# mlpc-ucsd/BDM

Hardware: AMD Instinct MI355X
Metric: sampled shapes/sec (4096 pts, 1000 DDPM steps) (higher is better)
Workload: dtype f32

## Files before the change

bdm_amd/csrc/pvconv_compact.hip:

```cpp
#include <stdlib.h>

#include "../../include/bdm_hip.h"
#include "common.h"
#include "se_fc.h"

using namespace bdm;

typedef __attribute__((ext_vector_type(8))) _Float16 f16x8;

namespace {

__device__ __forceinline__ void split2c(float v, unsigned short &h, unsigned short &l) {
  v = fminf(fmaxf(v, -65504.f), 65504.f);
  const _Float16 hi = (_Float16)v;
  const _Float16 lo = (_Float16)(v - (float)hi);
  h = __builtin_bit_cast(unsigned short, hi);
  l = __builtin_bit_cast(unsigned short, lo);
}

__device__ __forceinline__ void split_rec(const float v[8], uint4 &ph, uint4 &pl) {
  unsigned short h[8], l[8];
#pragma unroll
  for (int j = 0; j < 8; ++j) split2c(v[j], h[j], l[j]);
  ph.x = h[0] | (h[1] << 16); ph.y = h[2] | (h[3] << 16); ph.z = h[4] | (h[5] << 16); ph.w = h[6] | (h[7] << 16);
  pl.x = l[0] | (l[1] << 16); pl.y = l[2] | (l[3] << 16); pl.z = l[4] | (l[5] << 16); pl.w = l[6] | (l[7] << 16);
}

__device__ __forceinline__ void all_group_stats(const double *__restrict__ partial, int bi, int G, int S, double count, float eps,
                                                float *s_mean, float *s_rstd) {
  const int tid = threadIdx.x, l = tid & 31, gq = tid >> 5, per = blockDim.x >> 5;
  for (int g0 = 0; g0 < G; g0 += per) {
    const int g = g0 + gq;
    double a = 0.0, q = 0.0;
    if (g < G) {
      const double *pp = partial + ((size_t)bi * G + g) * S * 2;
      for (int sl = l; sl < S; sl += 32) { a += pp[2 * sl]; q += pp[2 * sl + 1]; }
    }
    a = half32_sum(a); q = half32_sum(q);
    if (l == 0 && g < G) {
      const double mu = a / count;
      double var = q / count - mu * mu;
      if (var < 0) var = 0;
      s_mean[g] = (float)mu;
      s_rstd[g] = (float)(1.0 / sqrt(var + (double)eps));
    }
  }
  __syncthreads();
}

}

__global__ __launch_bounds__(256) void to_h2_rows_kernel(int C, int V, int G, int S, int n_rows_max, int tiles_max, int dense_in,
                                                         const float *__restrict__ x, const int *__restrict__ dil_list,
                                                         const int *__restrict__ tile_start, const float *__restrict__ bias,
                                                         const double *__restrict__ partial, const float *__restrict__ gamma,
                                                         const float *__restrict__ beta, float eps, int act, float act_scale,
                                                         uint4 *__restrict__ rows_h2, uint4 *__restrict__ const_h2,
                                                         float *__restrict__ const_f32, unsigned *__restrict__ saturated) {
  __shared__ float s_mean[64], s_rstd[64];
  __shared__ float s_a[256], s_b[256];
  const int bi = blockIdx.y, tid = threadIdx.x, lane = tid & 63;
  const int C8 = (C + 7) / 8;
  const int nd = tile_start[((size_t)bi * tiles_max + tiles_max - 1) * 16 + 1];
  constexpr int RB = 512;
  if ((int)blockIdx.x * RB >= nd && blockIdx.x != 0) return;
  const int cg = C / G;
  const float g_pre = tid < C ? gamma[tid] : 0.f, b_pre = tid < C ? beta[tid] : 0.f;
  const int per_pass = blockDim.x / C8;
  const int c8 = tid % C8, rl = tid / C8;
  const int nch = min(8, C - c8 * 8);
  const bool vec = (C & 3) == 0 && nch == 8;
  auto load_row = [&](int j, float (&in)[8]) {
    if (dense_in) {
      const int v = dil_list[(size_t)bi * n_rows_max + j];
      const float *xb = x + ((size_t)bi * C + c8 * 8) * V + v;
#pragma unroll
      for (int u = 0; u < 8; ++u) in[u] = xb[(size_t)min(u, nch - 1) * V];
    } else {
      const float *row = x + ((size_t)bi * n_rows_max + j) * C + c8 * 8;
      if (vec) {
        const float4 p = *reinterpret_cast<const float4 *>(row), q = *reinterpret_cast<const float4 *>(row + 4);
        in[0] = p.x; in[1] = p.y; in[2] = p.z; in[3] = p.w; in[4] = q.x; in[5] = q.y; in[6] = q.z; in[7] = q.w;
      } else {
#pragma unroll
        for (int u = 0; u < 8; ++u) in[u] = row[min(u, nch - 1)];
      }
    }
  };
  const int j_end = min(nd, (int)(blockIdx.x + 1) * RB), j_first = blockIdx.x * RB + rl;
  const bool pre4 = rl < per_pass && j_first + 3 * per_pass < j_end;
  float pin0[8], pin1[8], pin2[8], pin3[8];
  if (pre4) { load_row(j_first, pin0); load_row(j_first + per_pass, pin1); load_row(j_first + 2 * per_pass, pin2); load_row(j_first + 3 * per_pass, pin3); }
  all_group_stats(partial, bi, G, S, (double)cg * V, eps, s_mean, s_rstd);
  for (int ch = tid; ch < C8 * 8; ch += blockDim.x) {
    float a = 0.f, bsh = 0.f;
    if (ch < C) {
      const int g = ch / cg;
      a = g_pre * s_rstd[g];
      bsh = b_pre - s_mean[g] * a;
    }
    s_a[ch] = a; s_b[ch] = bsh;
  }
  __syncthreads();
  bool sat = false;
  if (blockIdx.x == 0 && tid < C8) {
    const int c8 = tid, nch = min(8, C - c8 * 8);
    float fill[8];
#pragma unroll
    for (int j = 0; j < 8; ++j) {
      const int ch = c8 * 8 + j;
      float t = (ch < C && bias ? bias[ch] : 0.f) * s_a[ch] + s_b[ch];
      if (act == 1) t = swishf(t);
      fill[j] = ch < C ? t * act_scale : 0.f;
      sat |= !(fabsf(fill[j]) <= 65504.f);
    }
    uint4 ph, pl;
    split_rec(fill, ph, pl);
    const_h2[((size_t)bi * C8 + c8) * 2 + 0] = ph;
    const_h2[((size_t)bi * C8 + c8) * 2 + 1] = pl;
    const f16x8 hh = *reinterpret_cast<const f16x8 *>(&ph), ll = *reinterpret_cast<const f16x8 *>(&pl);
    for (int j = 0; j < nch; ++j) const_f32[(size_t)bi * C + c8 * 8 + j] = ((float)hh[j] + (float)ll[j]) * (1.0f / act_scale);
  }
  float ca[8], cb[8];
#pragma unroll
  for (int j = 0; j < 8; ++j) { ca[j] = s_a[c8 * 8 + j]; cb[j] = s_b[c8 * 8 + j]; }
  if (rl < per_pass) {
    auto emit_row = [&](int j, const float (&in)[8]) {
      float val[8];
#pragma unroll
      for (int u = 0; u < 8; ++u) {
        float t = in[u] * ca[u] + cb[u];
        if (act == 1) t = swishf(t);
        val[u] = t * act_scale;
        sat |= !(fabsf(val[u]) <= 65504.f);
      }
      uint4 ph, pl;
      split_rec(val, ph, pl);
      rows_h2[(((size_t)bi * C8 + c8) * 2 + 0) * n_rows_max + j] = ph;
      rows_h2[(((size_t)bi * C8 + c8) * 2 + 1) * n_rows_max + j] = pl;
    };
    int j = j_first;
    if (pre4) {
      emit_row(j, pin0); emit_row(j + per_pass, pin1); emit_row(j + 2 * per_pass, pin2); emit_row(j + 3 * per_pass, pin3);
      j += 4 * per_pass;
    }
    for (; j + 3 * per_pass < j_end; j += 4 * per_pass) {
      float in0[8], in1[8], in2[8], in3[8];
      load_row(j, in0); load_row(j + per_pass, in1); load_row(j + 2 * per_pass, in2); load_row(j + 3 * per_pass, in3);
      emit_row(j, in0); emit_row(j + per_pass, in1); emit_row(j + 2 * per_pass, in2); emit_row(j + 3 * per_pass, in3);
    }
    for (; j < j_end; j += per_pass) {
      float in0[8];
      load_row(j, in0);
      emit_row(j, in0);
    }
  }
  if (saturated != nullptr && __ballot(sat) != 0ull && lane == __ffsll((long long)__ballot(sat)) - 1) atomicOr(saturated, 1u);
}

extern "C" int bdm_group_norm_to_h2_rows(int b, int c, int v, int groups, const float *x, int dense_in, int n_rows_max,
                                         const int *dil_list, const int *tile_start, int tiles_max, const float *bias,
                                         const float *gamma, const float *beta, float eps, int act, float act_scale, void *rows_h2,
                                         void *const_h2, float *const_f32, const void *partial, int slices,
                                         unsigned int *saturated, void *stream) {
  BDM_REQUIRE(b >= 0 && c >= 1 && c <= 256 && v >= 1 && groups >= 1 && groups <= 64 && c % groups == 0 && (c / groups) >= 4 &&
                  partial != nullptr && slices >= 1 && x != nullptr && dil_list != nullptr && tile_start != nullptr && tiles_max >= 1 &&
                  n_rows_max >= 1 && rows_h2 && const_h2 && const_f32,
              "group_norm_to_h2_rows: bad arguments (<= 256 channels)");
  {
    int ex = 0;
    BDM_REQUIRE(act_scale > 0.f && act_scale < INFINITY && frexpf(act_scale, &ex) == 0.5f,
                "group_norm_to_h2_rows: act_scale must be a power of two (got %g)", (double)act_scale);
  }
  if (b == 0) return BDM_OK;
  dim3 grid(cdiv(n_rows_max, 512), b);
  hipLaunchKernelGGL(to_h2_rows_kernel, grid, dim3(256), 0, (hipStream_t)stream, c, v, groups, slices, n_rows_max, tiles_max, dense_in, x,
                     dil_list, tile_start, bias, (const double *)partial, gamma, beta, eps, act, act_scale, (uint4 *)rows_h2,
                     (uint4 *)const_h2, const_f32, saturated);
  return launch_status("group_norm_to_h2_rows");
}

__global__ void class_weight_sums_kernel(int cout, int cin, const float *__restrict__ w, double *__restrict__ wsum) {
  const long long total = 27ll * cin * cout;
  for (long long e = (long long)blockIdx.x * blockDim.x + threadIdx.x; e < total; e += (long long)gridDim.x * blockDim.x) {
    const int co = (int)(e % cout), ci = (int)((e / cout) % cin), k = (int)(e / ((long long)cout * cin));
    const int cls[3] = {k / 9, (k / 3) % 3, k % 3};
    double a = 0.0;
    for (int t = 0; t < 27; ++t) {
      const int d[3] = {t / 9 - 1, (t / 3) % 3 - 1, t % 3 - 1};
      bool in = true;
      for (int ax = 0; ax < 3; ++ax) in = in && !(cls[ax] == 0 && d[ax] == -1) && !(cls[ax] == 2 && d[ax] == 1);
      if (in) a += (double)w[((size_t)co * cin + ci) * 27 + t];
    }
    wsum[e] = a;
  }
}
extern "C" size_t bdm_conv3d_class_weight_elems(int cout, int cin) { return (size_t)27 * cin * cout; }
extern "C" int bdm_conv3d_class_weight_sums(int cout, int cin, const float *w, void *wsum, void *stream) {
  BDM_REQUIRE(cout >= 1 && cin >= 1 && w != nullptr && wsum != nullptr, "conv3d_class_weight_sums: bad arguments");
  hipLaunchKernelGGL(class_weight_sums_kernel, dim3(256), dim3(256), 0, (hipStream_t)stream, cout, cin, w, (double *)wsum);
  return launch_status("conv3d_class_weight_sums");
}

__global__ __launch_bounds__(256) void class_constants_kernel(int cin, int cout, const double *__restrict__ wsum, const float *__restrict__ bias,
                                                              const float *__restrict__ const_f32, const int *__restrict__ class_count,
                                                              float *__restrict__ class_vals, int G, int S, int slice0,
                                                              double *__restrict__ gn_partial) {
  __shared__ float s_c[256];
  __shared__ float s_v[256];
  const int k = blockIdx.x, bi = blockIdx.y, tid = threadIdx.x;
  for (int ci = tid; ci < cin; ci += blockDim.x) s_c[ci] = const_f32[(size_t)bi * cin + ci];
  __syncthreads();
  const double *wk = wsum + (size_t)k * cin * cout;
  for (int co = tid; co < cout; co += blockDim.x) {
    double a = bias ? (double)bias[co] : 0.0;
#pragma unroll 8
    for (int ci = 0; ci < cin; ++ci) a += wk[(size_t)ci * cout + co] * (double)s_c[ci];
    const float v = (float)a;
    class_vals[((size_t)bi * 27 + k) * cout + co] = v;
    s_v[co] = v;
  }
  __syncthreads();
  if (gn_partial != nullptr && tid < G) {
    const int cg = cout / G;
    double a = 0.0, q = 0.0;
    for (int j = 0; j < cg; ++j) { const double v = (double)s_v[tid * cg + j]; a += v; q += v * v; }
    const double n = (double)class_count[(size_t)bi * 27 + k];
    double *dst = gn_partial + (((size_t)bi * G + tid) * S + slice0 + k) * 2;
    dst[0] = n * a;
    dst[1] = n * q;
  }
}
extern "C" int bdm_conv3d_class_constants(int b, int cin, int cout, const void *wsum, const float *bias, const float *const_f32,
                                          const int *class_count, float *class_vals, int groups, void *gn_partial, int slices,
                                          int slice0, void *stream) {
  BDM_REQUIRE(b >= 0 && cin >= 1 && cin <= 256 && cout >= 1 && cout <= 256 && wsum && const_f32 && class_count && class_vals,
              "conv3d_class_constants: bad arguments (<= 256 channels)");
  BDM_REQUIRE(gn_partial == nullptr || (groups >= 1 && groups <= 64 && cout % groups == 0 && slice0 >= 0 && slice0 + 27 <= slices),
              "conv3d_class_constants: bad GroupNorm slice arguments");
  if (b == 0) return BDM_OK;
  hipLaunchKernelGGL(class_constants_kernel, dim3(27, b), dim3(256), 0, (hipStream_t)stream, cin, cout, (const double *)wsum, bias, const_f32,
                     class_count, class_vals, groups, slices, slice0, (double *)gn_partial);
  return launch_status("conv3d_class_constants");
}

#define SE_SLABS 64
struct GnFoldC {
  const double *partial;
  int S, G, l;
  const float *gamma, *beta;
  float eps;
};

__global__ __launch_bounds__(256) void se_rows_partial_kernel(int c, int V, int G, int S, int n_rows_max, int tiles_max,
                                                              const float *__restrict__ rows, const int *__restrict__ tile_start,
                                                              const double *__restrict__ partial, const float *__restrict__ gamma,
                                                              const float *__restrict__ beta, float eps, float2 *__restrict__ coef,
                                                              float *__restrict__ part, GnFoldC pf, float2 *__restrict__ pf_coef) {
  __shared__ float s_mean[64], s_rstd[64];
  __shared__ float s_a[256], s_b[256];
  __shared__ float s_acc[256];
  const int slab = blockIdx.x, bi = blockIdx.y, tid = threadIdx.x;
  const int cg = c / G;
  all_group_stats(partial, bi, G, S, (double)cg * V, eps, s_mean, s_rstd);
  for (int ch = tid; ch < c; ch += blockDim.x) {
    const float ga = gamma[ch] * s_rstd[ch / cg];
    s_a[ch] = ga;
    s_b[ch] = beta[ch] - s_mean[ch / cg] * ga;
  }
  __syncthreads();
  if (slab == 0) {
    for (int ch = tid; ch < c; ch += blockDim.x) coef[(size_t)bi * c + ch] = make_float2(s_a[ch], s_b[ch]);
    if (pf.partial != nullptr) {
      const int cgp = c / pf.G;
      for (int ch = tid; ch < c; ch += blockDim.x) {
        const int gp = ch / cgp;
        double a = 0.0, q = 0.0;
        const double *p = pf.partial + ((size_t)bi * pf.G + gp) * pf.S * 2;
        for (int s = 0; s < pf.S; ++s) { a += p[2 * s]; q += p[2 * s + 1]; }
        const double cnt = (double)cgp * pf.l, mu = a / cnt;
        double var = q / cnt - mu * mu;
        if (var < 0) var = 0;
        const float ga = pf.gamma[ch] * (float)(1.0 / sqrt(var + (double)pf.eps));
        pf_coef[(size_t)bi * c + ch] = make_float2(ga, pf.beta[ch] - (float)mu * ga);
// ... 226 lines not shown
```

bdm_amd/modules.py:

```python
import os
from typing import NamedTuple

import torch
import torch.nn as nn

from . import functional as F
from . import ops
from . import tape

__all__ = ["Swish", "SharedMLP", "SE3d", "Voxelization", "Attention", "PVConv", "BallQuery",
           "PointNetSAModule", "PointNetFPModule"]


class Swish(nn.Module):

    def forward(self, x):
        raise RuntimeError("Swish is fused into bdm_group_norm on the HIP path")


class SharedMLP(nn.Module):

    def __init__(self, in_channels, out_channels, dim=1):
        super().__init__()
        if dim == 1:
# ... 376 lines not shown
        if route.plan_args is None:
            assert col_bias is None
            self._need_features(features)
            if route.first == "dense_s3":
                norm_coords, vox_coords = ops.voxel_coords(coords, r, self.voxelization.eps)
                x3 = ops.avg_voxelize_s3(features, vox_coords, r)
                return _VoxelBranch(ops.conv3d_s3(x3, self._packed_weight(conv1, "bf16x6"), conv1.bias, conv1.in_channels, cout, r), None, None, norm_coords)
            vox, norm_coords = self.voxelization(features, coords, with_row_occupancy=r >= 32)
            vox, rowocc = vox if r >= 32 else (vox, None)
            return _VoxelBranch(ops.conv3d(vox, self._packed_weight(conv1, "fp32"), conv1.bias, r, rowocc=rowocc), None, None, norm_coords)
        plan = ops.voxel_plan(coords, *route.plan_args)
        groups = gn1.num_groups if route.want_stats else None
        if route.first == "map":
            v = ops.sparse_first_conv_from_map(self._hoisted(features), plan, conv1, cout, gn_groups=groups)
        else:
            self._need_features(features)
            if route.first == "dil":
                v = ops.sparse_first_conv_os(features, plan, self._packed_weight(conv1, "fp16x3"), conv1.bias, cout, gn_groups=groups,
                                             compact=route.compact_first)
            else:
                impl = route.gemm_impl
                rows = rows_in if (route.takes_rows and rows_in.plan is plan and rows_in.channels == conv1.in_channels) else None
                if route.first == "gemm_split":
                    xh = ops.sparse_first_conv_planned(features, plan, self._packed_weight(conv1, impl), conv1.bias, cout, rows=rows, impl=impl,
                                                       h2_out=(gn1, ops.h2_activation_scale(gn1), ops.saturation_slot(self, features.device)))
                    return _VoxelBranch(None, None, plan, plan.norm_coords, xh)
                cin = features.shape[1] if col_bias is not None else None
                v = ops.sparse_first_conv_planned(features, plan, self._packed_weight(conv1, impl, cin=cin), conv1.bias, cout,
                                                  gn_groups=groups, rows=rows, col_bias=col_bias, impl=impl)
        return _VoxelBranch(*(v if groups else (v, None)), plan, plan.norm_coords)

    def _second_conv(self, route, vb):
        r = self.resolution
        _, gn1, conv2, gn2, _, _ = self._parts()
        cin, cout = conv2.in_channels, conv2.out_channels
        if route.second == "fp32":
            ops.group_norm_(vb.v, gn1.weight, gn1.bias, 8, gn1.eps, swish=True)
            vb.v = ops.conv3d(vb.v, self._packed_weight(conv2, "fp32"), conv2.bias, r)
        elif route.second == "bf16x6":
            vb.v = ops.conv3d_s3(ops.to_s3(vb.v, gn1, swish=True), self._packed_weight(conv2, "bf16x6"), conv2.bias, cin, cout, r)
        else:
            if vb.xh is None:
                sat = ops.saturation_slot(self, vb.v.device) if vb.v.is_cuda else None
                vb.xh = ops.to_h2(vb.v, gn1, swish=True, saturated=sat, stats=vb.gn1_stats)
            if route.tail == "plain":
                vb.v = ops.conv3d_h2(vb.xh, self._packed_weight(conv2, "fp16x3"), conv2.bias, cin, cout, r)
            else:
                vb.v, vb.stats = ops.conv3d_h2_gn(vb.xh, self._packed_weight(conv2, "fp16x3"), conv2.bias, cin, cout, r, gn2.num_groups)

    def _tail_lists(self, route, vb, pf, pf_ready, pf_pending):
        conv1, gn1, conv2, gn2, _, se = self._parts()
        plan, norm_coords = vb.plan, vb.norm_coords
        sat = ops.saturation_slot(self, pf.device)
        rows_h2, const_h2, const_f32, inv_s = ops.to_h2_rows(vb.v, plan, gn1, vb.gn1_stats, saturated=sat, bias=conv1.bias)
        y2, cvals, st2 = ops.second_conv_rows(rows_h2, const_h2, const_f32, inv_s, plan, self._packed_weight(conv2, "fp16x3"),
                                              self._packed_weight(conv2, "class"), conv2.bias, conv2.in_channels,
                                              conv2.out_channels, gn2.num_groups)
        w1, w2 = se.fc[0].weight, se.fc[2].weight
        if pf_pending is not None:
            if pf_ready is not None:
                tape.wait_event(pf_ready)
            gate, coef, pf_coef = ops.se_gate_gn_rows(y2, cvals, plan, st2, gn2, w1, w2, pf=pf_pending, n_points=pf.shape[2])
            return ops.devoxelize_gn_gate_add_rows(norm_coords, y2, cvals, plan, coef, gate=gate, add=pf, add_coef=pf_coef)
        gate, coef = ops.se_gate_gn_rows(y2, cvals, plan, st2, gn2, w1, w2)
        if pf_ready is not None:
            tape.wait_event(pf_ready)
        return ops.devoxelize_gn_gate_add_rows(norm_coords, y2, cvals, plan, coef, gate=gate, add=pf)

    def _tail_small(self, route, vb, pf, pf_ready, pf_pending):
        _, _, conv2, gn2, _, se = self._parts()
        head = None
        if route.head:
            head = vb.plan, ops.h2_sum_scale([gn2, self.point_features.layers[-2]]), ops.saturation_slot(self._next_pv, pf.device)
        if pf_ready is not None:
            tape.wait_event(pf_ready)
        pf_coef = None
        if pf_pending is not None:
            mean, coef, pf_coef = ops.se_means_gn(vb.v, vb.stats, gn2, pf=pf_pending, n_points=pf.shape[2])
        else:
            mean, coef = ops.se_means_gn(vb.v, vb.stats, gn2)
        out, rows = ops.pvconv_tail_small(vb.norm_coords, vb.v, coef, mean, se.fc[0].weight, se.fc[2].weight, self.resolution, add=pf, add_coef=pf_coef,
                                          head=head)
        if rows is not None:
            out._bdm_rows = rows
        return out

    def _tail_se_devox(self, route, vb, pf, pf_ready, pf_pending):
        _, _, _, gn2, _, se = self._parts()
        mean, coef = ops.se_means_gn(vb.v, vb.stats, gn2)
        if pf_ready is not None:
            tape.wait_event(pf_ready)
        return ops.devoxelize_gn_se_add(vb.norm_coords, vb.v, coef, self.resolution, mean, se.fc[0].weight, se.fc[2].weight, add=pf)

    def _tail_folded(self, route, vb, pf, pf_ready, pf_pending):
        _, _, _, gn2, _, se = self._parts()
        w1, w2 = se.fc[0].weight, se.fc[2].weight
        v, stats, norm_coords = vb.v, vb.stats, vb.norm_coords
        if pf_pending is not None:
            if pf_ready is not None:
                tape.wait_event(pf_ready)
            gate, coef, pf_coef = ops.se_gate_gn(v, stats, gn2, w1, w2, pf=pf_pending, n_points=pf.shape[2])
            return ops.devoxelize_gn_gate_add(norm_coords, v, coef, self.resolution, gate=gate, add=pf, add_coef=pf_coef)
        gate, coef = ops.se_gate_gn(v, stats, gn2, w1, w2)
        if pf_ready is not None:
            tape.wait_event(pf_ready)
        return ops.devoxelize_gn_gate_add(norm_coords, v, coef, self.resolution, gate=gate, add=pf)

    def _tail_plain(self, route, vb, pf, pf_ready, pf_pending):
        _, _, _, gn2, att, se = self._parts()
        ops.group_norm_(vb.v, gn2.weight, gn2.bias, 8, gn2.eps, swish=(att is None))
# ... 250 lines not shown
```

bdm_amd/ops.py:

```python
import ctypes
import os

import torch

from . import _lib as L
from . import tape


def _bcl(t):
    if t.dtype != torch.float32:
        raise L.BdmHipError(f"expected float32, got {t.dtype}")
    B, C = t.shape[0], t.shape[1]
    if B * C > 0 and t.is_contiguous():
        l = t.numel() // (B * C)
        return t, B, C, l, C * l, l
    l = 1
    for s in t.shape[2:]:
        l *= s
    dense, exp = True, 1
    for d in range(t.dim() - 1, 1, -1):
        if t.shape[d] != 1 and t.stride(d) != exp:
            dense = False
        exp *= t.shape[d]
    if dense and C > 1 and t.stride(1) < l:
# ... 1158 lines not shown
            L.check(fn(nb, plan.n_max, C, 27 * cout, L.ptr(xs[b0:]), L.ptr(wt), L.ptr(plan.n_occ[b0:]), *cb, L.ptr(y), L.stream()), name[4:])
    return _gather_groups(plan, B, cout, bias, gn_groups, gemm, gb, y, out)


def sparse_conv_pack_os(weight, form="dil"):
    return (form,) + tuple(conv3d_h2_pack(weight))


class CompactGrid:

    def __init__(self, rows, plan, bias, channels):
        self.rows, self.plan, self.bias, self.channels = rows, plan, bias, channels

    is_cuda = property(lambda self: self.rows.is_cuda)
    device = property(lambda self: self.rows.device)

    def dense(self):
        B, r3, C = self.rows.shape[0], self.plan.r ** 3, self.channels
        out = self.bias.detach().view(1, C, 1).expand(B, C, r3).contiguous()
        idx = self.plan.dil_index.long()
        for b in range(B):
            v = torch.nonzero(idx[b] >= 0).squeeze(1)
            out[b, :, v] = self.rows[b, idx[b, v]].t()
        return out


def sparse_first_conv_os(features, plan, packed, bias, cout, gn_groups=None, compact=False):
    plan_dilation(plan)
    if plan.dil_list is None:
        raise L.BdmHipError(f"sparse_first_conv_os: resolution {plan.r} has no dilated plan (8, 16, 32)")
    f, B, C, n, bs_f, ld_f = _bcl(features)
    dev, lib, r = f.device, L.lib(), plan.r
    packed_w, inv_scale = packed
    xr, slots = _records_f32((f, B, C, n, bs_f, ld_f), plan, extra=1)
    amax, counter = slots[:B], slots[B:]
    if compact:
        y = torch.empty(B, plan.n_dil_max, cout, dtype=torch.float32, device=dev)
        out = CompactGrid(y, plan, bias, cout)
    else:
        y = out = torch.empty(B, cout, r ** 3, dtype=torch.float32, device=dev)
    args = (B, C, cout, r, plan.n_max, plan.n_dil_max, L.ptr(xr), L.ptr(amax), L.ptr(plan.occ_index), L.ptr(plan.dil_list),
            L.ptr(plan.dil_index), L.ptr(plan.tile_start), L.ptr(packed_w), L.ptr(inv_scale), L.ptr(bias), L.ptr(y), 1 if compact else 0)
    if gn_groups:
        tiles = plan.tile_start.shape[1]
        partial = torch.empty(B, gn_groups, tiles, 2, dtype=torch.float64, device=dev)
        slices = ctypes.c_int(0)
        L.check(lib.bdm_sparse_conv_dil_gn(*args, int(gn_groups), L.ptr(partial), ctypes.byref(slices), plan.tile, L.ptr(counter), L.stream()),
                "sparse_conv_dil_gn")
        return out, (partial, tiles, int(gn_groups))
    L.check(lib.bdm_sparse_conv_dil(*args, plan.tile, L.ptr(counter), L.stream()), "sparse_conv_dil")
    return out


def to_h2_rows(x, plan, gn, stats, swish=True, saturated=None, bias=None):
    plan_dilation(plan)
    lib = L.lib()
    compact = isinstance(x, CompactGrid)
    src = x.rows if compact else x.contiguous()
    bias = x.bias if compact else bias
    B, C, V = src.shape[0], (x.channels if compact else src.shape[1]), plan.r ** 3
    dev = src.device
    s = float(h2_activation_scale(gn))
    C8 = (C + 7) // 8
    rows = torch.empty(B, C8, 2, plan.n_dil_max, 8, dtype=torch.float16, device=dev)
    const_h2 = torch.empty(B, C8, 2, 8, dtype=torch.float16, device=dev)
    const_f32 = torch.empty(B, C, dtype=torch.float32, device=dev)
    partial, slices, groups = stats
    L.check(lib.bdm_group_norm_to_h2_rows(B, C, V, groups, L.ptr(src), 0 if compact else 1, plan.n_dil_max, L.ptr(plan.dil_list),
                                          L.ptr(plan.tile_start), plan.tile_start.shape[1], L.ptr(bias), L.ptr(gn.weight), L.ptr(gn.bias),
                                          L.c_float(gn.eps), 1 if swish else 0, L.c_float(s), L.ptr(rows), L.ptr(const_h2), L.ptr(const_f32),
                                          L.ptr(partial), slices, L.ptr(saturated), L.stream()), "group_norm_to_h2_rows")
    return rows, const_h2, const_f32, 1.0 / s


def conv_class_pack(weight):
    cout, cin = weight.shape[:2]
    lib = L.lib()
    wsum = torch.empty(lib.bdm_conv3d_class_weight_elems(cout, cin), dtype=torch.float64, device=weight.device)
    L.check(lib.bdm_conv3d_class_weight_sums(cout, cin, L.ptr(weight.contiguous()), L.ptr(wsum), L.stream()), "conv3d_class_weight_sums")
    return wsum


def second_conv_rows(rows_h2, const_h2, const_f32, x_inv_scale, plan, packed, wsum, bias, cin, cout, groups=8):
    plan_dilation2(plan)
    lib, B, r = L.lib(), rows_h2.shape[0], plan.r
    dev = rows_h2.device
    packed_w, inv_scale = packed
    y = torch.empty(B, plan.n_dil_max, cout, dtype=torch.float32, device=dev)
    tiles = plan.d2_tiles.shape[1]
    partial = torch.empty(B, groups, tiles + 27, 2, dtype=torch.float64, device=dev)
    counter = amax_slots(dev, 1)
    slices = ctypes.c_int(0)
    L.check(lib.bdm_sparse_conv_dil_h2_gn(B, cin, cout, r, plan.n_dil_max, plan.n_dil_max, L.ptr(rows_h2), L.ptr(const_h2), L.c_float(x_inv_scale),
                                          L.ptr(plan.dil_index), L.ptr(plan.d2_list), L.ptr(plan.d2_index), L.ptr(plan.d2_tiles), L.ptr(packed_w),
                                          L.ptr(inv_scale), L.ptr(bias), L.ptr(y), int(groups), L.ptr(partial), ctypes.byref(slices), plan.d2_tile,
                                          L.ptr(counter), L.stream()), "sparse_conv_dil_h2_gn")
    assert slices.value == tiles + 27
    class_vals = torch.empty(B, 27, cout, dtype=torch.float32, device=dev)
    L.check(lib.bdm_conv3d_class_constants(B, cin, cout, L.ptr(wsum), L.ptr(bias), L.ptr(const_f32), L.ptr(plan.d2_class_count), L.ptr(class_vals),
                                           int(groups), L.ptr(partial), tiles + 27, tiles, L.stream()), "conv3d_class_constants")
    return y, class_vals, (partial, tiles + 27)


def se_gate_gn_rows(rows, class_vals, plan, stats, gn, w1, w2, pf=None, n_points=0):
    partial, slices = stats
    B, C = rows.shape[0], rows.shape[2]
    dev, lib = rows.device, L.lib()
    V = plan.r ** 3
    mean = torch.empty(B, C, dtype=torch.float32, device=dev)
    coef = torch.empty(B, C, 2, dtype=torch.float32, device=dev)
    gate = torch.empty(B, C, dtype=torch.float32, device=dev)
    part = torch.empty(lib.bdm_se_gate_gn_rows_workspace_elems(B, C), dtype=torch.float32, device=dev)
    args = (B, C, w1.shape[0], V, gn.num_groups, L.ptr(rows), plan.n_dil_max, L.ptr(plan.d2_tiles), plan.d2_tiles.shape[1], L.ptr(class_vals),
            L.ptr(plan.d2_class_count), L.ptr(partial), slices, L.ptr(gn.weight), L.ptr(gn.bias), L.c_float(gn.eps), L.ptr(w1), L.ptr(w2), L.ptr(part),
            L.ptr(mean), L.ptr(coef), L.ptr(gate))
    if pf is not None:
        (pp, ps, pg), pgn = pf
        pf_coef = torch.empty(B, C, 2, dtype=torch.float32, device=dev)
        L.check(lib.bdm_se_gate_gn_rows_pf(*args, L.ptr(pp), ps, pg, int(n_points), L.ptr(pgn.weight), L.ptr(pgn.bias), L.c_float(pgn.eps),
                                           L.ptr(pf_coef), L.stream()), "se_gate_gn_rows_pf")
        return gate, coef, pf_coef
    L.check(lib.bdm_se_gate_gn_rows(*args, L.stream()), "se_gate_gn_rows")
    return gate, coef


def devoxelize_gn_gate_add_rows(norm_coords, rows, class_vals, plan, coef, gate=None, add=None, add_coef=None):
    B, C = rows.shape[0], rows.shape[2]
    n = norm_coords.shape[2]
    out = torch.empty(B, C, n, dtype=torch.float32, device=rows.device)
    _, _, _, _, bs_o, ld_o = _bcl(out)
    bs_a, ld_a = _addend_strides(add)
    lib = L.lib()
    args = (B, C, n, plan.r, L.ptr(norm_coords), L.ptr(rows), plan.n_dil_max, L.ptr(plan.d2_index), L.ptr(class_vals), L.ptr(coef), L.ptr(gate),
            L.ptr(add), bs_a, ld_a)
    if add_coef is not None:
        L.check(lib.bdm_devoxelize_gn_gate_add_rows_pf(*args, L.ptr(add_coef), L.ptr(out), bs_o, ld_o, L.stream()), "devoxelize_gn_gate_add_rows_pf")
    else:
        L.check(lib.bdm_devoxelize_gn_gate_add_rows(*args, L.ptr(out), bs_o, ld_o, L.stream()), "devoxelize_gn_gate_add_rows")
    return out


def densify_rows(rows, class_vals, plan):
    B, _, C = rows.shape
    r = plan.r
    ax = torch.arange(r, device=rows.device)
    cls1 = torch.where(ax == 0, 0, torch.where(ax == r - 1, 2, 1))
    cls = (cls1[:, None, None] * 9 + cls1[None, :, None] * 3 + cls1[None, None, :]).reshape(-1)
    out = class_vals[:, cls].permute(0, 2, 1).contiguous()
    idx = plan.d2_index.long()
    for b in range(B):
# ... 49 lines not shown
```

bdm_amd/pvcnn.py:

```python
import os

import torch
import torch.nn as nn

from . import ops
from . import tape
from .modules import Attention, PointNetFPModule, PointNetSAModule, PVConv, SharedMLP

SA_BLOCKS = [
    ((32, 2, 32), (1024, 0.1, 32, (32, 64))),
    ((64, 3, 16), (256, 0.2, 32, (64, 128))),
    ((128, 3, 8), (64, 0.4, 32, (128, 256))),
    (None, (16, 0.8, 32, (256, 256, 512))),
]
FP_BLOCKS = [
    ((256, 256), (256, 3, 8)),
    ((256, 256), (256, 3, 8)),
    ((256, 128), (128, 2, 16)),
    ((128, 128, 64), (64, 2, 32)),
]


def create_pointnet2_sa_components(sa_blocks, extra_feature_channels, embed_dim=64, use_att=False, dropout=0.1,
                                   with_se=False, normalize=True, eps=0, width_multiplier=1,
# ... 93 lines not shown
SIDE_STREAM_PRIORITY = int(os.environ.get("BDM_SIDE_PRIORITY", "0"))
DEFER_CHAIN = True
SIDE_NN = True
NN_PLANS = {}


EARLY_SAMPLER = os.environ.get("BDM_EARLY_SAMPLER", "1") == "1"


def _side_stream(device):
    cur = torch.cuda.current_stream(device)
    key = (device, cur.cuda_stream)
    side = _side_streams.get(key)
    if side is None:
        side = _side_streams[key] = torch.cuda.Stream(device=device, priority=SIDE_STREAM_PRIORITY)
    return cur, side


def early_first_sampler(net, x_t):
    sa_layers = getattr(net, "sa_layers", None)
    if not (EARLY_SAMPLER and SIDE_STREAM and sa_layers is not None and x_t.is_cuda and x_t.dim() == 3 and x_t.shape[2] == 3
            and x_t.shape[0] * x_t.shape[1] >= SIDE_STREAM_MIN_POINTS):
        return None
    first = sa_layers[0][-1] if isinstance(sa_layers[0], nn.Sequential) else sa_layers[0]
    cur, side = _side_stream(x_t.device)
    tape.wait_stream(side, cur)
    with torch.cuda.stream(side):
        c0 = ops.transpose12(x_t) if x_t.is_contiguous() else x_t.transpose(1, 2).contiguous()
        centers0 = first.sample(c0)
    return (c0, centers0, side)


def plan_sampling_chain(sa_layers, coords, early=None, fp_layers=None):
    cur, side = _side_stream(coords.device)
    tape.wait_stream(side, cur)
    first = sa_layers[0][-1] if isinstance(sa_layers[0], nn.Sequential) else sa_layers[0]
    c0 = coords.contiguous()
    if early is not None and early[2] is side and tuple(early[0].shape) == tuple(c0.shape) and early[1].shape[2] == first.num_centers:
        centers0 = early[1]
    else:
        with torch.cuda.stream(side):
            centers0 = first.sample(c0)

    def level(li, c, centers):
        sa = sa_layers[li][-1] if isinstance(sa_layers[li], nn.Sequential) else sa_layers[li]
        if li > 0:
            centers = sa.sample(c)
        idx = sa.query(c, centers)
        ev = torch.cuda.Event()
        tape.record_event(ev, side)
        sa._planned = (centers, idx, ev, c if li > 0 else coords)
        nxt = sa_layers[li + 1] if li + 1 < len(sa_layers) else None
        if SIDE_PLAN and isinstance(nxt, nn.Sequential) and isinstance(nxt[0], PVConv):
            plan_ahead(nxt[0], centers)
        return centers

    def plan_ahead(pv, points, unless_cached=False):
        route = pv.route(points.shape[0], points.shape[2])
        if route.plan_args is not None and not (unless_cached and ops.has_voxel_plan(points, route.plan_args[0])):
            plan = ops.voxel_plan(points, *route.plan_args, dilate=route.dilate)
            plan.ready = torch.cuda.Event()
            tape.record_event(plan.ready, side)

    wanted = {}
    for i, blk in enumerate(fp_layers if fp_layers is not None else ()):
        pv = next((m for m in blk if isinstance(m, PVConv)), None) if isinstance(blk, nn.Sequential) else None
        if pv is not None and SIDE_PLAN and DECODER_PLAN:
            wanted[i] = pv

    def remaining(c):
        with torch.cuda.stream(side):
            cents = [c]
            for li in range(1, len(sa_layers)):
                c = level(li, c, None)
                cents.append(c)
                if li + 1 < len(sa_layers):
                    if len(sa_layers) - 2 - li in wanted:
                        plan_ahead(wanted[len(sa_layers) - 2 - li], c, unless_cached=True)
            if SIDE_NN:
                chain = [c0] + cents
                for pts, ctr in zip(chain[:-1], chain[1:]):
                    idx, w = ops.three_nn_search(pts, ctr)
                    ev = torch.cuda.Event()
                    tape.record_event(ev, side)
                    NN_PLANS[(pts.data_ptr(), ctr.data_ptr())] = (pts, ctr, idx, w, ev)

    def rest():
        with torch.cuda.stream(side):
            c1 = level(0, c0, centers0)
        first._more = lambda: remaining(c1)
        return first._planned

    if DEFER_CHAIN:
        first._planned = (rest, coords)
    else:
        rest()
        more, first._more = first._more, None
        more()


def encode(sa_layers, global_att, inputs, t_emb, early=None, fp_layers=None):
    coords = ops.xyz_rows(inputs)
    ops.clear_plan_cache()
    NN_PLANS.clear()
    for blocks in sa_layers:
        (blocks[-1] if isinstance(blocks, nn.Sequential) else blocks)._planned = None
        (blocks[-1] if isinstance(blocks, nn.Sequential) else blocks)._more = None
        first = blocks[0] if isinstance(blocks, nn.Sequential) else blocks
        if getattr(first, "_temb_terms", None) is not None:
            first._temb_terms = None
    if coords.is_cuda and SIDE_STREAM and coords.shape[0] * coords.shape[2] >= SIDE_STREAM_MIN_POINTS:
        plan_sampling_chain(sa_layers, coords, early, fp_layers)
    features = inputs
    coords_list, in_features_list = [], []
    for i, sa_blocks in enumerate(sa_layers):
        in_features_list.append(features)
        coords_list.append(coords)
        if i == 0:
            features, coords, t_emb = run_blocks(sa_blocks, (features, coords, t_emb))
        else:
            first = sa_blocks[0] if isinstance(sa_blocks, nn.Sequential) else sa_blocks
            can = hasattr(first, "can_split_temb") and first.can_split_temb(features, t_emb)
            if can and i == 1:
                _enc_temb_terms(sa_layers, t_emb)
            if not can and hasattr(first, "_temb_terms"):
                first._temb_terms = None
            features, coords, t_emb = run_blocks(sa_blocks, (features if can else ops.cat_channels([features, t_emb]), coords, t_emb))
    if global_att is not None:
        features = global_att(features)
    return features, coords, t_emb, coords_list, in_features_list

# ... 212 lines not shown
```

include/bdm_hip.h:

```cpp
#ifndef BDM_HIP_H
#define BDM_HIP_H

#include <stddef.h>
#include <stdint.h>

#ifdef __cplusplus
extern "C" {
#endif

const char *bdm_last_error(void);
int bdm_abi_version(void);


int bdm_furthest_point_sampling(int b, int n, int m, const float *coords, int *indices,
                                float *centers_out, void *stream);

int bdm_gather_features_forward(int b, int c, int n, int m, const float *features,
                                const int *indices, float *out, void *stream);

int bdm_ball_query(int b, int n, int m, float radius, int u, const float *centers,
                   const float *points, int *neighbors, void *stream);

int bdm_grouping_forward(int b, int c, int n, int m, int u, const float *features,
                         const int *indices, float *out, void *stream);
// ... 215 lines not shown

int bdm_voxel_compact(int b, int r, int n_max, const int *cnt, int *occ_index, int *occ_list, int *n_occ,
                      void *stream);
int bdm_sparse_voxel_features(int b, int c, int n, int r, int n_max, const float *features, long long bs_f,
                              int ld_f, const int *cnt, const void *plan_workspace, const int *occ_list,
                              const int *n_occ, float *xc, void *stream);
int bdm_sparse_conv_pack_weights(int cout, int cin, const float *w, float *wt, void *stream);
int bdm_sparse_conv_gemm(int b, int n_max, int cin, int n27, const float *xc, const float *wt,
                         const int *n_occ, float *y, void *stream);
int bdm_sparse_conv_gather(int b, int cout, int r, int n_max, const float *y, const int *occ_index,
                           const unsigned char *rowocc, const float *bias, float *out, void *stream);
int bdm_sparse_conv_gather_gn(int b, int cout, int r, int n_max, const float *y, const int *occ_index,
                              const unsigned char *rowocc, const float *bias, float *out, int groups, void *gn_partial,
                              void *stream);

int bdm_sparse_voxel_features_f32(int b, int c, int n, int r, int n_max, const float *features, long long bs_f,
                                  int ld_f, const int *cnt, const void *plan_workspace, const int *occ_list,
                                  const int *n_occ, void *xr, float *amax, void *stream);
#ifdef BDM_EXPERIMENTAL
size_t bdm_sparse_conv_fused_weight_elems(int cout, int cin);
int bdm_sparse_conv_fused_pack_weights(int cout, int cin, const float *w, void *packed, float *scale_ws,
                                       float *inv_scale, void *stream);
int bdm_sparse_conv_fused(int b, int cin, int cout, int r, int n_max, const void *xr, const float *amax,
                          const void *packed_w, const float *inv_scale, const int *occ_list, const int *n_occ,
                          const float *bias, float *out, void *stream);
#endif

size_t bdm_sparse_conv_h2_weight_elems(int cout, int cin);
int bdm_sparse_conv_pack_weights_h2(int cout, int cin, const float *w, void *packed, float *scale_ws,
                                    float *inv_scale, void *stream);
int bdm_sparse_split_h2(int b, int cin, int n_max, const void *xr, const float *amax, void *xh, void *stream);
int bdm_sparse_conv_gemm_h2(int b, int n_max, int cin, int cout, const void *xh, const float *amax, const void *packed_w,
                            const float *inv_scale, const int *n_occ, float *y, void *stream);
int bdm_sparse_conv_gemm_h2_cb(int b, int n_max, int cin, int cout, const void *xh, const float *amax, const void *packed_w,
                               const float *inv_scale, const int *n_occ, const float *col_bias, long long bs_cb, float *y, void *stream);

int bdm_voxel_dilate_slices(int r, int tile);
int bdm_voxel_dilate(int b, int r, int n_dil_max, const int *cnt, int *dil_list, int *dil_index, int *plane_start, int *tile_start,
                     int tile, void *stream);
int bdm_sparse_conv_dil(int b, int cin, int cout, int r, int n_max, int n_dil_max, const void *xr, const float *amax,
                        const int *occ_index, const int *dil_list, const int *dil_index, const int *tile_start,
                        const void *packed_w, const float *inv_scale, const float *bias, float *y, int compact, int tile,
                        int *work_counter, void *stream);
int bdm_sparse_conv_dil_gn(int b, int cin, int cout, int r, int n_max, int n_dil_max, const void *xr, const float *amax,
                           const int *occ_index, const int *dil_list, const int *dil_index, const int *tile_start,
                           const void *packed_w, const float *inv_scale, const float *bias, float *y, int compact, int groups,
                           void *gn_partial, int *slices_out, int tile, int *work_counter, void *stream);

int bdm_voxel_dilate_again(int b, int r, int n_dil_max, const int *dil_index_in, int *dil_list, int *dil_index, int *plane_start,
                           int *tile_start, int *class_count, int tile, void *stream);
int bdm_group_norm_to_h2_rows(int b, int c, int v, int groups, const float *x, int dense_in, int n_rows_max, const int *dil_list,
                              const int *tile_start, int tiles_max, const float *bias, const float *gamma, const float *beta,
                              float eps, int act, float act_scale, void *rows_h2, void *const_h2, float *const_f32,
                              const void *partial, int slices, unsigned int *saturated, void *stream);
int bdm_sparse_conv_dil_h2_gn(int b, int cin, int cout, int r, int n_rows_max, int n_dil_max, const void *rows_h2, const void *xconst,
                              float x_inv_scale, const int *in_index, const int *dil_list, const int *dil_index,
                              const int *tile_start, const void *packed_w, const float *inv_scale, const float *bias, float *y,
                              int groups, void *gn_partial, int *slices_out, int tile, int *work_counter, void *stream);
size_t bdm_conv3d_class_weight_elems(int cout, int cin);
int bdm_conv3d_class_weight_sums(int cout, int cin, const float *w, void *wsum, void *stream);
int bdm_conv3d_class_constants(int b, int cin, int cout, const void *wsum, const float *bias, const float *const_f32,
                               const int *class_count, float *class_vals, int groups, void *gn_partial, int slices, int slice0,
                               void *stream);
size_t bdm_se_gate_gn_rows_workspace_elems(int b, int c);
int bdm_se_gate_gn_rows(int b, int c, int hidden, int v, int groups, const float *rows, int n_rows_max, const int *tile_start,
                        int tiles_max, const float *class_vals, const int *class_count, const void *gn_partial, int slices,
                        const float *gamma, const float *beta, float eps, const float *w1, const float *w2, float *part_ws,
                        float *mean_ws, float *coef, float *gate, void *stream);
int bdm_se_gate_gn_rows_pf(int b, int c, int hidden, int v, int groups, const float *rows, int n_rows_max, const int *tile_start,
                           int tiles_max, const float *class_vals, const int *class_count, const void *gn_partial, int slices,
                           const float *gamma, const float *beta, float eps, const float *w1, const float *w2, float *part_ws,
                           float *mean_ws, float *coef, float *gate, const void *pf_partial, int pf_slices, int pf_groups, int pf_n,
                           const float *pf_gamma, const float *pf_beta, float pf_eps, float *pf_coef, void *stream);
int bdm_devoxelize_gn_gate_add_rows(int b, int c, int n, int r, const float *coords, const float *rows, int n_rows_max,
                                    const int *dil_index, const float *class_vals, const float *coef, const float *gate,
                                    const float *add, long long bs_a, int ld_a, float *out, long long bs_o, int ld_o, void *stream);
int bdm_devoxelize_gn_gate_add_rows_pf(int b, int c, int n, int r, const float *coords, const float *rows, int n_rows_max,
                                       const int *dil_index, const float *class_vals, const float *coef, const float *gate,
                                       const float *add, long long bs_a, int ld_a, const float *add_coef, float *out, long long bs_o,
                                       int ld_o, void *stream);


int bdm_ddpm_step(long long n, const float *x, const float *eps, const float *noise,
                  float sqrt_beta_prod, float sqrt_alpha_prod, float coef_x0, float coef_x,
                  float sigma, float *out, void *stream);
int bdm_ddpm_step_dev(long long n, const float *x, const float *eps, const float *noise, const float *coef,
                      float *out, void *stream);

int bdm_ddim_step(long long n, const float *x, const float *eps, const float *noise, float sqrt_beta_prod,
                  float sqrt_alpha_prod, float coef_x0, float coef_eps, float sigma, float *out, void *stream);

int bdm_lincomb(long long n, int k, float c0, const float *x0, float c1, const float *x1, float c2,
                const float *x2, float c3, const float *x3, float div, float *out, void *stream);

int bdm_pvd_step(long long n, const float *x, const float *eps, const float *noise,
                 float sqrt_recip_abar, float sqrt_recipm1_abar, float coef1, float coef2,
                 float sigma, float *out, void *stream);

int bdm_philox_normal(int b, long long per_shape, const unsigned long long *keys, unsigned int draw,
                      unsigned int purpose, float *out, void *stream);
int bdm_philox_bits(int b, long long per_shape, const unsigned long long *keys, unsigned int draw,
                    unsigned int purpose, long long *out, void *stream);
int bdm_ddpm_step_philox(int b, long long per_shape, const float *x, const float *eps,
                         const unsigned long long *keys, unsigned int draw, unsigned int purpose,
                         float sqrt_beta_prod, float sqrt_alpha_prod, float coef_x0, float coef_x, float sigma,
                         float *out, void *stream);
int bdm_pvd_step_philox(int b, long long per_shape, const float *x, const float *eps,
// ... 85 lines not shown
```

Baseline: 2.963.

## Fuse class-constant computation into group-norm-to-h2 rows kernel and share voxel plans

Adds 27 extra blocks per batch to the to_h2_rows kernel. They recompute the GroupNorm affine and the constant fill, then compute the conv2 class constants and their GroupNorm partials, so the separate conv3d_class_constants launch after the second conv is no longer needed. Separately, plan-ahead now takes the maximum dilation over PVConv layers that share the same plan arguments, so a single voxel plan can serve encoder and decoder layers. This removes one kernel launch and one serialization point per block, at the cost of redundant group-stats work in the extra blocks and possibly larger dilated plans.

```diff
diff --git a/bdm_amd/csrc/pvconv_compact.hip b/bdm_amd/csrc/pvconv_compact.hip
--- a/bdm_amd/csrc/pvconv_compact.hip
+++ b/bdm_amd/csrc/pvconv_compact.hip
@@ -48,6 +48,57 @@
   __syncthreads();
 }
 
+__device__ __forceinline__ bool const_chunk(int C, int c8, const float *__restrict__ bias, const float *s_a, const float *s_b, int act,
+                                            float act_scale, uint4 &ph, uint4 &pl, float (&f32)[8]) {
+  bool sat = false;
+  float fill[8];
+#pragma unroll
+  for (int j = 0; j < 8; ++j) {
+    const int ch = c8 * 8 + j;
+    float t = (ch < C && bias ? bias[ch] : 0.f) * s_a[ch] + s_b[ch];
+    if (act == 1) t = swishf(t);
+    fill[j] = ch < C ? t * act_scale : 0.f;
+    sat |= !(fabsf(fill[j]) <= 65504.f);
+  }
+  split_rec(fill, ph, pl);
+  const f16x8 hh = *reinterpret_cast<const f16x8 *>(&ph), ll = *reinterpret_cast<const f16x8 *>(&pl);
+#pragma unroll
+  for (int j = 0; j < 8; ++j) f32[j] = ((float)hh[j] + (float)ll[j]) * (1.0f / act_scale);
+  return sat;
+}
+
+struct ClassConst {
+  int cout;
+  const double *wsum;
+  const float *bias;
+  const int *class_count;
+  float *class_vals;
+  int G, S, slice0;
+  double *gn_partial;
+};
+__device__ __forceinline__ void class_constants_body(int k, int bi, int cin, const ClassConst &cc, const float *s_c, float *s_v) {
+  const int tid = threadIdx.x, cout = cc.cout;
+  const double *wk = cc.wsum + (size_t)k * cin * cout;
+  for (int co = tid; co < cout; co += blockDim.x) {
+    double a = cc.bias ? (double)cc.bias[co] : 0.0;
+#pragma unroll 8
+    for (int ci = 0; ci < cin; ++ci) a += wk[(size_t)ci * cout + co] * (double)s_c[ci];
+    const float v = (float)a;
+    cc.class_vals[((size_t)bi * 27 + k) * cout + co] = v;
+    s_v[co] = v;
+  }
+  __syncthreads();
+  if (cc.gn_partial != nullptr && tid < cc.G) {
+    const int cg = cout / cc.G;
+    double a = 0.0, q = 0.0;
+    for (int j = 0; j < cg; ++j) { const double v = (double)s_v[tid * cg + j]; a += v; q += v * v; }
+    const double n = (double)cc.class_count[(size_t)bi * 27 + k];
+    double *dst = cc.gn_partial + (((size_t)bi * cc.G + tid) * cc.S + cc.slice0 + k) * 2;
+    dst[0] = n * a;
+    dst[1] = n * q;
+  }
+}
+
 }
 
 __global__ __launch_bounds__(256) void to_h2_rows_kernel(int C, int V, int G, int S, int n_rows_max, int tiles_max, int dense_in,
@@ -56,11 +107,38 @@
                                                          const double *__restrict__ partial, const float *__restrict__ gamma,
                                                          const float *__restrict__ beta, float eps, int act, float act_scale,
                                                          uint4 *__restrict__ rows_h2, uint4 *__restrict__ const_h2,
-                                                         float *__restrict__ const_f32, unsigned *__restrict__ saturated) {
+                                                         float *__restrict__ const_f32, unsigned *__restrict__ saturated,
+                                                         int row_blocks, ClassConst cc) {
   __shared__ float s_mean[64], s_rstd[64];
   __shared__ float s_a[256], s_b[256];
   const int bi = blockIdx.y, tid = threadIdx.x, lane = tid & 63;
   const int C8 = (C + 7) / 8;
+  if ((int)blockIdx.x >= row_blocks) {
+    __shared__ float s_c[256], s_v[256];
+    const int cg = C / G;
+    const float g_pre = tid < C ? gamma[tid] : 0.f, b_pre = tid < C ? beta[tid] : 0.f;
+    all_group_stats(partial, bi, G, S, (double)cg * V, eps, s_mean, s_rstd);
+    for (int ch = tid; ch < C8 * 8; ch += blockDim.x) {
+      float a = 0.f, bsh = 0.f;
+      if (ch < C) {
+        const int g = ch / cg;
+        a = g_pre * s_rstd[g];
+        bsh = b_pre - s_mean[g] * a;
+      }
+      s_a[ch] = a; s_b[ch] = bsh;
+    }
+    __syncthreads();
+    if (tid < C8) {
+      uint4 ph, pl;
+      float f32[8];
+      (void)const_chunk(C, tid, bias, s_a, s_b, act, act_scale, ph, pl, f32);
+      const int nch = min(8, C - tid * 8);
+      for (int j = 0; j < nch; ++j) s_c[tid * 8 + j] = f32[j];
+    }
+    __syncthreads();
+    class_constants_body((int)blockIdx.x - row_blocks, bi, C, cc, s_c, s_v);
+    return;
+  }
   const int nd = tile_start[((size_t)bi * tiles_max + tiles_max - 1) * 16 + 1];
   constexpr int RB = 512;
   if ((int)blockIdx.x * RB >= nd && blockIdx.x != 0) return;
@@ -105,21 +183,12 @@
   bool sat = false;
   if (blockIdx.x == 0 && tid < C8) {
     const int c8 = tid, nch = min(8, C - c8 * 8);
-    float fill[8];
-#pragma unroll
-    for (int j = 0; j < 8; ++j) {
-      const int ch = c8 * 8 + j;
-      float t = (ch < C && bias ? bias[ch] : 0.f) * s_a[ch] + s_b[ch];
-      if (act == 1) t = swishf(t);
-      fill[j] = ch < C ? t * act_scale : 0.f;
-      sat |= !(fabsf(fill[j]) <= 65504.f);
-    }
     uint4 ph, pl;
-    split_rec(fill, ph, pl);
+    float f32[8];
+    sat |= const_chunk(C, c8, bias, s_a, s_b, act, act_scale, ph, pl, f32);
     const_h2[((size_t)bi * C8 + c8) * 2 + 0] = ph;
     const_h2[((size_t)bi * C8 + c8) * 2 + 1] = pl;
-    const f16x8 hh = *reinterpret_cast<const f16x8 *>(&ph), ll = *reinterpret_cast<const f16x8 *>(&pl);
-    for (int j = 0; j < nch; ++j) const_f32[(size_t)bi * C + c8 * 8 + j] = ((float)hh[j] + (float)ll[j]) * (1.0f / act_scale);
+    for (int j = 0; j < nch; ++j) const_f32[(size_t)bi * C + c8 * 8 + j] = f32[j];
   }
   float ca[8], cb[8];
 #pragma unroll
@@ -162,7 +231,9 @@
                                          const int *dil_list, const int *tile_start, int tiles_max, const float *bias,
                                          const float *gamma, const float *beta, float eps, int act, float act_scale, void *rows_h2,
                                          void *const_h2, float *const_f32, const void *partial, int slices,
-                                         unsigned int *saturated, void *stream) {
+                                         unsigned int *saturated, int cls_cout, const void *cls_wsum, const float *cls_bias,
+                                         const int *class_count, float *class_vals, int cls_groups, void *cls_gn_partial,
+                                         int cls_slices, int cls_slice0, void *stream) {
   BDM_REQUIRE(b >= 0 && c >= 1 && c <= 256 && v >= 1 && groups >= 1 && groups <= 64 && c % groups == 0 && (c / groups) >= 4 &&
                   partial != nullptr && slices >= 1 && x != nullptr && dil_list != nullptr && tile_start != nullptr && tiles_max >= 1 &&
                   n_rows_max >= 1 && rows_h2 && const_h2 && const_f32,
@@ -172,11 +243,20 @@
     BDM_REQUIRE(act_scale > 0.f && act_scale < INFINITY && frexpf(act_scale, &ex) == 0.5f,
                 "group_norm_to_h2_rows: act_scale must be a power of two (got %g)", (double)act_scale);
   }
+  ClassConst cc{};
+  if (cls_wsum != nullptr) {
+    BDM_REQUIRE(cls_cout >= 1 && cls_cout <= 256 && class_count && class_vals, "group_norm_to_h2_rows: bad class-constant arguments (<= 256 channels)");
+    BDM_REQUIRE(cls_gn_partial == nullptr || (cls_groups >= 1 && cls_groups <= 64 && cls_cout % cls_groups == 0 && cls_slice0 >= 0 &&
+                                              cls_slice0 + 27 <= cls_slices),
+                "group_norm_to_h2_rows: bad GroupNorm slice arguments of the class constants");
+    cc = ClassConst{cls_cout, (const double *)cls_wsum, cls_bias, class_count, class_vals, cls_groups, cls_slices, cls_slice0, (double *)cls_gn_partial};
+  }
   if (b == 0) return BDM_OK;
-  dim3 grid(cdiv(n_rows_max, 512), b);
+  const int row_blocks = cdiv(n_rows_max, 512);
+  dim3 grid(row_blocks + (cls_wsum != nullptr ? 27 : 0), b);
   hipLaunchKernelGGL(to_h2_rows_kernel, grid, dim3(256), 0, (hipStream_t)stream, c, v, groups, slices, n_rows_max, tiles_max, dense_in, x,
                      dil_list, tile_start, bias, (const double *)partial, gamma, beta, eps, act, act_scale, (uint4 *)rows_h2,
-                     (uint4 *)const_h2, const_f32, saturated);
+                     (uint4 *)const_h2, const_f32, saturated, row_blocks, cc);
   return launch_status("group_norm_to_h2_rows");
 }
 
@@ -211,25 +291,7 @@
   const int k = blockIdx.x, bi = blockIdx.y, tid = threadIdx.x;
   for (int ci = tid; ci < cin; ci += blockDim.x) s_c[ci] = const_f32[(size_t)bi * cin + ci];
   __syncthreads();
-  const double *wk = wsum + (size_t)k * cin * cout;
-  for (int co = tid; co < cout; co += blockDim.x) {
-    double a = bias ? (double)bias[co] : 0.0;
-#pragma unroll 8
-    for (int ci = 0; ci < cin; ++ci) a += wk[(size_t)ci * cout + co] * (double)s_c[ci];
-    const float v = (float)a;
-    class_vals[((size_t)bi * 27 + k) * cout + co] = v;
-    s_v[co] = v;
-  }
-  __syncthreads();
-  if (gn_partial != nullptr && tid < G) {
-    const int cg = cout / G;
-    double a = 0.0, q = 0.0;
-    for (int j = 0; j < cg; ++j) { const double v = (double)s_v[tid * cg + j]; a += v; q += v * v; }
-    const double n = (double)class_count[(size_t)bi * 27 + k];
-    double *dst = gn_partial + (((size_t)bi * G + tid) * S + slice0 + k) * 2;
-    dst[0] = n * a;
-    dst[1] = n * q;
-  }
+  class_constants_body(k, bi, cin, ClassConst{cout, wsum, bias, class_count, class_vals, G, S, slice0, gn_partial}, s_c, s_v);
 }
 extern "C" int bdm_conv3d_class_constants(int b, int cin, int cout, const void *wsum, const float *bias, const float *const_f32,
                                           const int *class_count, float *class_vals, int groups, void *gn_partial, int slices,
diff --git a/bdm_amd/modules.py b/bdm_amd/modules.py
--- a/bdm_amd/modules.py
+++ b/bdm_amd/modules.py
@@ -452,10 +452,11 @@
         conv1, gn1, conv2, gn2, _, se = self._parts()
         plan, norm_coords = vb.plan, vb.norm_coords
         sat = ops.saturation_slot(self, pf.device)
-        rows_h2, const_h2, const_f32, inv_s = ops.to_h2_rows(vb.v, plan, gn1, vb.gn1_stats, saturated=sat, bias=conv1.bias)
-        y2, cvals, st2 = ops.second_conv_rows(rows_h2, const_h2, const_f32, inv_s, plan, self._packed_weight(conv2, "fp16x3"),
-                                              self._packed_weight(conv2, "class"), conv2.bias, conv2.in_channels,
-                                              conv2.out_channels, gn2.num_groups)
+        wsum = self._packed_weight(conv2, "class")
+        rows_h2, const_h2, const_f32, inv_s, class_done = ops.to_h2_rows(vb.v, plan, gn1, vb.gn1_stats, saturated=sat, bias=conv1.bias,
+                                                                         class_consts=(wsum, conv2.bias, conv2.out_channels, gn2.num_groups))
+        y2, cvals, st2 = ops.second_conv_rows(rows_h2, const_h2, const_f32, inv_s, plan, self._packed_weight(conv2, "fp16x3"), wsum, conv2.bias,
+                                              conv2.in_channels, conv2.out_channels, gn2.num_groups, class_done=class_done)
         w1, w2 = se.fc[0].weight, se.fc[2].weight
         if pf_pending is not None:
             if pf_ready is not None:
diff --git a/bdm_amd/ops.py b/bdm_amd/ops.py
--- a/bdm_amd/ops.py
+++ b/bdm_amd/ops.py
@@ -1234,7 +1234,7 @@
     return out
 
 
-def to_h2_rows(x, plan, gn, stats, swish=True, saturated=None, bias=None):
+def to_h2_rows(x, plan, gn, stats, swish=True, saturated=None, bias=None, class_consts=None):
     plan_dilation(plan)
     lib = L.lib()
     compact = isinstance(x, CompactGrid)
@@ -1248,10 +1248,19 @@
     const_h2 = torch.empty(B, C8, 2, 8, dtype=torch.float16, device=dev)
     const_f32 = torch.empty(B, C, dtype=torch.float32, device=dev)
     partial, slices, groups = stats
+    cls, done = (0, None, None, None, None, 0, None, 0, 0), None
+    if class_consts is not None:
+        wsum, bias2, cout, groups2 = class_consts
+        plan_dilation2(plan)
+        tiles = plan.d2_tiles.shape[1]
+        done = (torch.empty(B, 27, cout, dtype=torch.float32, device=dev), torch.empty(B, groups2, tiles + 27, 2, dtype=torch.float64, device=dev))
+        cls = (int(cout), L.ptr(wsum), L.ptr(bias2), L.ptr(plan.d2_class_count), L.ptr(done[0]), int(groups2), L.ptr(done[1]), tiles + 27, tiles)
     L.check(lib.bdm_group_norm_to_h2_rows(B, C, V, groups, L.ptr(src), 0 if compact else 1, plan.n_dil_max, L.ptr(plan.dil_list),
                                           L.ptr(plan.tile_start), plan.tile_start.shape[1], L.ptr(bias), L.ptr(gn.weight), L.ptr(gn.bias),
                                           L.c_float(gn.eps), 1 if swish else 0, L.c_float(s), L.ptr(rows), L.ptr(const_h2), L.ptr(const_f32),
-                                          L.ptr(partial), slices, L.ptr(saturated), L.stream()), "group_norm_to_h2_rows")
+                                          L.ptr(partial), slices, L.ptr(saturated), *cls, L.stream()), "group_norm_to_h2_rows")
+    if done is not None:
+        return rows, const_h2, const_f32, 1.0 / s, done
     return rows, const_h2, const_f32, 1.0 / s
 
 
@@ -1263,14 +1272,15 @@
     return wsum
 
 
-def second_conv_rows(rows_h2, const_h2, const_f32, x_inv_scale, plan, packed, wsum, bias, cin, cout, groups=8):
+def second_conv_rows(rows_h2, const_h2, const_f32, x_inv_scale, plan, packed, wsum, bias, cin, cout, groups=8, class_done=None):
     plan_dilation2(plan)
     lib, B, r = L.lib(), rows_h2.shape[0], plan.r
     dev = rows_h2.device
     packed_w, inv_scale = packed
     y = torch.empty(B, plan.n_dil_max, cout, dtype=torch.float32, device=dev)
     tiles = plan.d2_tiles.shape[1]
-    partial = torch.empty(B, groups, tiles + 27, 2, dtype=torch.float64, device=dev)
+    class_vals, partial = class_done if class_done is not None else (None, torch.empty(B, groups, tiles + 27, 2, dtype=torch.float64, device=dev))
+    assert tuple(partial.shape) == (B, groups, tiles + 27, 2)
     counter = amax_slots(dev, 1)
     slices = ctypes.c_int(0)
     L.check(lib.bdm_sparse_conv_dil_h2_gn(B, cin, cout, r, plan.n_dil_max, plan.n_dil_max, L.ptr(rows_h2), L.ptr(const_h2), L.c_float(x_inv_scale),
@@ -1278,6 +1288,8 @@
                                           L.ptr(inv_scale), L.ptr(bias), L.ptr(y), int(groups), L.ptr(partial), ctypes.byref(slices), plan.d2_tile,
                                           L.ptr(counter), L.stream()), "sparse_conv_dil_h2_gn")
     assert slices.value == tiles + 27
+    if class_done is not None:
+        return y, class_vals, (partial, tiles + 27)
     class_vals = torch.empty(B, 27, cout, dtype=torch.float32, device=dev)
     L.check(lib.bdm_conv3d_class_constants(B, cin, cout, L.ptr(wsum), L.ptr(bias), L.ptr(const_f32), L.ptr(plan.d2_class_count), L.ptr(class_vals),
                                            int(groups), L.ptr(partial), tiles + 27, tiles, L.stream()), "conv3d_class_constants")
diff --git a/bdm_amd/pvcnn.py b/bdm_amd/pvcnn.py
--- a/bdm_amd/pvcnn.py
+++ b/bdm_amd/pvcnn.py
@@ -169,13 +169,20 @@
         sa._planned = (centers, idx, ev, c if li > 0 else coords)
         nxt = sa_layers[li + 1] if li + 1 < len(sa_layers) else None
         if SIDE_PLAN and isinstance(nxt, nn.Sequential) and isinstance(nxt[0], PVConv):
-            plan_ahead(nxt[0], centers)
+            dec = fp_layers[len(sa_layers) - 2 - li] if fp_layers is not None and 0 <= len(sa_layers) - 2 - li < len(fp_layers) else None
+            plan_ahead(nxt[0], centers, sharers=list(nxt) + (list(dec) if isinstance(dec, nn.Sequential) else []))
         return centers
 
-    def plan_ahead(pv, points, unless_cached=False):
+    def plan_ahead(pv, points, unless_cached=False, sharers=()):
         route = pv.route(points.shape[0], points.shape[2])
         if route.plan_args is not None and not (unless_cached and ops.has_voxel_plan(points, route.plan_args[0])):
-            plan = ops.voxel_plan(points, *route.plan_args, dilate=route.dilate)
+            dilate = route.dilate
+            for m in sharers:
+                if isinstance(m, PVConv) and m is not pv and m.resolution == pv.resolution:
+                    other = m.route(points.shape[0], points.shape[2])
+                    if other.plan_args == route.plan_args:
+                        dilate = max(dilate, other.dilate)
+            plan = ops.voxel_plan(points, *route.plan_args, dilate=dilate)
             plan.ready = torch.cuda.Event()
             tape.record_event(plan.ready, side)
 
@@ -193,7 +200,7 @@
                 cents.append(c)
                 if li + 1 < len(sa_layers):
                     if len(sa_layers) - 2 - li in wanted:
-                        plan_ahead(wanted[len(sa_layers) - 2 - li], c, unless_cached=True)
+                        plan_ahead(wanted[len(sa_layers) - 2 - li], c, unless_cached=True, sharers=list(fp_layers[len(sa_layers) - 2 - li]))
             if SIDE_NN:
                 chain = [c0] + cents
                 for pts, ctr in zip(chain[:-1], chain[1:]):
diff --git a/include/bdm_hip.h b/include/bdm_hip.h
--- a/include/bdm_hip.h
+++ b/include/bdm_hip.h
@@ -291,7 +291,9 @@
 int bdm_group_norm_to_h2_rows(int b, int c, int v, int groups, const float *x, int dense_in, int n_rows_max, const int *dil_list,
                               const int *tile_start, int tiles_max, const float *bias, const float *gamma, const float *beta,
                               float eps, int act, float act_scale, void *rows_h2, void *const_h2, float *const_f32,
-                              const void *partial, int slices, unsigned int *saturated, void *stream);
+                              const void *partial, int slices, unsigned int *saturated, int cls_cout, const void *cls_wsum,
+                              const float *cls_bias, const int *class_count, float *class_vals, int cls_groups,
+                              void *cls_gn_partial, int cls_slices, int cls_slice0, void *stream);
 int bdm_sparse_conv_dil_h2_gn(int b, int cin, int cout, int r, int n_rows_max, int n_dil_max, const void *rows_h2, const void *xconst,
                               float x_inv_scale, const int *in_index, const int *dil_list, const int *dil_index,
                               const int *tile_start, const void *packed_w, const float *inv_scale, const float *bias, float *y,
```

New measurement: 2.985 (median of 6 runs). About the same (+0.7%).
